# ChangUk/RecommenderSystems

Hardware: AMD Instinct MI355X
Metric: RWR seeds/sec + achieved HBM GB/s on 100M-edge bipartite graph, 1/2/4/8 GPUs (higher is better)
Workload: dtype f64

## Files before the change

### recommendersystems_amd/csrc/iterate.hip

```cpp
#include "iterate.h"

#include <climits>
#include <cstdlib>
#include <type_traits>

namespace rwr {

template <int G, bool VF>
__global__ __launch_bounds__(256) void k_spmm(int32_t n, const int64_t *__restrict__ in_ptr,
                                              const int32_t *__restrict__ in_src,
                                              const double *__restrict__ in_w,
                                              const int32_t *__restrict__ row_order, int32_t nrows,
                                              const double *__restrict__ X, double *__restrict__ Y,
                                              const int32_t *__restrict__ seeds, double c1, int skip_seed_row,
                                              const double *__restrict__ w_src, double *__restrict__ Zout)
{
    constexpr int RPW = WAVE / G;
    constexpr int U = 4;
    const int tile = blockIdx.y;
    const size_t toff = (size_t)tile * (size_t)n * G;
    X += toff;
    Y += toff;
    if (VF && Zout) Zout += toff;
    const int lane = threadIdx.x & (WAVE - 1);
    const int sub = lane / G, k = lane % G;
    const int32_t my_seed = skip_seed_row ? seeds[tile * G + k] : -1;
    const int wpb = blockDim.x / WAVE;
    const int64_t nwaves = (int64_t)gridDim.x * wpb;
    for (int64_t rb = ((int64_t)blockIdx.x * wpb + threadIdx.x / WAVE) * RPW; rb < nrows; rb += nwaves * RPW) {
        const int64_t r = rb + sub;
        int32_t j = -1;
        int64_t p = 0, e = 0;
        if (r < nrows) {
            j = row_order[r];
            p = in_ptr[j];
            e = in_ptr[j + 1];
        }
        double acc = 0.0;
        for (; p + U <= e; p += U) {
            int32_t idx[U];
            double wv[U], xv[U];
#pragma unroll
            for (int u = 0; u < U; ++u) idx[u] = in_src[p + u];
#pragma unroll
            for (int u = 0; u < U; ++u) wv[u] = VF ? 0.0 : in_w[p + u];
#pragma unroll
            for (int u = 0; u < U; ++u) xv[u] = X[(size_t)idx[u] * G + k];
#pragma unroll
            for (int u = 0; u < U; ++u) {
                if (VF) {
                    acc += xv[u];
                } else {
                    double rw = c1 * xv[u];
                    acc += rw * wv[u];
                }
            }
        }
        for (; p < e; ++p) {
            if (VF) {
                acc += X[(size_t)in_src[p] * G + k];
            } else {
                double rw = c1 * X[(size_t)in_src[p] * G + k];
                acc += rw * in_w[p];
            }
        }
        if (j >= 0 && j != my_seed) {
            Y[(size_t)j * G + k] = acc;
            if (VF && Zout) { const double rw = c1 * acc; Zout[(size_t)j * G + k] = rw * w_src[j]; }
        }
    }
}

template <int G, int CH, bool CHECK, bool WRITE, bool VF, bool SEL = false>
__device__ __forceinline__ void spmm_chunked_body(int32_t n, const int64_t *__restrict__ in_ptr,
                                                  const int32_t *__restrict__ in_src,
                                                  const double *__restrict__ in_w,
                                                  const int32_t *__restrict__ row_order, int32_t nrows,
                                                  const double *__restrict__ X, double *__restrict__ Y,
                                                  const int32_t *__restrict__ seeds, double c1,
                                                  int skip_seed_row, const uint32_t *__restrict__ nz_in,
                                                  uint32_t *__restrict__ nz_out,
                                                  const uint32_t *__restrict__ act,
                                                  const double *__restrict__ w_src, double *__restrict__ Zout,
                                                  const SelSink sink = SelSink{})
{
    static_assert(G >= 8 && G <= 64, "chunked SpMM needs 8 <= G <= 64");
    static_assert(!SEL || (!CHECK && !WRITE), "the selecting form probes and writes no bitmap");
    constexpr int RPW = WAVE / G;
    const int tile = blockIdx.y;
    const size_t toff = (size_t)tile * (size_t)n * G;
    X += toff;
    if (!SEL) Y += toff;
    if (VF && Zout) Zout += toff;
    const size_t nzw = ((size_t)n + 31) / 32;
    if (CHECK) nz_in += (size_t)tile * nzw;
    if (WRITE) nz_out += (size_t)tile * nzw;
    if (CHECK && act) act += (size_t)tile * nzw;
    const int lane = threadIdx.x & (WAVE - 1);
    const int sub = lane / G, k = lane % G;
    const int gbase = (lane - k) << 2;
    const int32_t my_seed = skip_seed_row ? seeds[tile * G + k] : -1;
    bool sel_real = false;
    double sel_tau = 0.0;
    if (SEL) {
        sel_real = seeds[tile * G + k] >= 0;
        sel_tau = sink.tau[tile * G + k];
    }
    const int wpb = blockDim.x / WAVE;
    const int64_t nwaves = (int64_t)gridDim.x * wpb;
    for (int64_t rb = ((int64_t)blockIdx.x * wpb + threadIdx.x / WAVE) * RPW; rb < nrows; rb += nwaves * RPW) {
        const int64_t r = rb + sub;
        int32_t j = -1;
        int64_t p = 0, e = 0;
        if (r < nrows) {
            j = row_order[r];
            p = in_ptr[j];
            e = in_ptr[j + 1];
            if (CHECK && act && !((act[(uint32_t)j >> 5] >> (j & 31)) & 1u)) e = p;
        }
        double acc = 0.0;
        while (__any(p < e)) {
            const int64_t left = e - p;
            const int cnt = left > CH ? CH : (left > 0 ? (int)left : 0);
            int32_t my_idx = 0;
            double my_w = 0.0;
            if (k < cnt) {
                my_idx = in_src[p + k];
                if (!VF) my_w = in_w[p + k];
                if (CHECK) {
                    const uint32_t wd = nz_in[(uint32_t)my_idx >> 5];
                    if (!((wd >> (my_idx & 31)) & 1u)) my_idx |= (int32_t)0x80000000;
                }
            }
            const int wlo = __double2loint(my_w), whi = __double2hiint(my_w);
            if (CHECK) {
                const unsigned long long lm = __ballot(k < cnt && my_idx >= 0);
                unsigned long long um = lm;
                if (G < 64) {
#pragma unroll
                    for (int sh = G; sh < 64; sh <<= 1) um |= um >> sh;
                    um &= (1ull << (G & 63)) - 1ull;
                }
                if (__popcll(um) <= 4) {
                    while (um) {
                        const int t = __builtin_ctzll(um);
                        um &= um - 1;
                        const int idx = __builtin_amdgcn_ds_bpermute(gbase + (t << 2), my_idx);
                        if (VF) {
                            if (t < cnt && idx >= 0) acc += X[(size_t)idx * G + k];
                        } else {
                            const int lo = __builtin_amdgcn_ds_bpermute(gbase + (t << 2), wlo);
                            const int hi = __builtin_amdgcn_ds_bpermute(gbase + (t << 2), whi);
                            if (t < cnt && idx >= 0) {
                                const double rw = c1 * X[(size_t)idx * G + k];
                                acc += rw * __hiloint2double(hi, lo);
                            }
                        }
                    }
                    p += cnt;
                    continue;
                }
            }
            double xv[CH], wv[CH];
#pragma unroll
            for (int t = 0; t < CH; ++t) {
                const int idx = __builtin_amdgcn_ds_bpermute(gbase + (t << 2), my_idx);
                if (!VF) {
                    const int lo = __builtin_amdgcn_ds_bpermute(gbase + (t << 2), wlo);
                    const int hi = __builtin_amdgcn_ds_bpermute(gbase + (t << 2), whi);
                    wv[t] = __hiloint2double(hi, lo);
                }
                xv[t] = (t < cnt && idx >= 0) ? X[(size_t)idx * G + k] : 0.0;
            }
#pragma unroll
            for (int t = 0; t < CH; ++t) {
                if (t < cnt) {
                    if (VF) {
                        acc += xv[t];
                    } else {
                        double rw = c1 * xv[t];
                        acc += rw * wv[t];
                    }
                }
            }
            p += cnt;
        }
        if constexpr (SEL) {
            if (j >= 0 && j != my_seed && sel_real && acc >= sel_tau) {
                const int slot = tile * G + k;
                const int32_t at = atomicAdd(&sink.cursor[slot], 1);
                if (at < sink.cap) sink.cand[(size_t)slot * (size_t)sink.stride + (size_t)at] = RowScore{j, 0, acc};
                else *sink.overflow = 1;
            }
        } else if (j >= 0 && j != my_seed) {
            Y[(size_t)j * G + k] = acc;
            if (VF && Zout) { const double rw = c1 * acc; Zout[(size_t)j * G + k] = rw * w_src[j]; }
        }
        if (WRITE) {
            const unsigned long long nzb = __ballot(acc != 0.0);
            const unsigned long long gmask = (G == 64) ? ~0ull : (((1ull << (G & 63)) - 1ull) << (sub * G));
            if (k == 0 && j >= 0 && (nzb & gmask)) atomicOr(&nz_out[(uint32_t)j >> 5], 1u << (j & 31));
        }
    }
}

template <int G, int CH, bool CHECK, bool WRITE, bool VF, bool LIST>
__global__ __launch_bounds__(256) void k_spmm_chunked(int32_t n, const int64_t *__restrict__ in_ptr,
                                                      const int32_t *__restrict__ in_src,
                                                      const double *__restrict__ in_w,
                                                      const int32_t *__restrict__ row_order, int32_t nrows,
                                                      const double *__restrict__ X, double *__restrict__ Y,
                                                      const int32_t *__restrict__ seeds, double c1,
                                                      int skip_seed_row, const uint32_t *__restrict__ nz_in,
                                                      uint32_t *__restrict__ nz_out,
                                                      const uint32_t *__restrict__ act,
                                                      const double *__restrict__ w_src, double *__restrict__ Zout)
{
    spmm_chunked_body<G, CH, CHECK, WRITE, VF>(n, in_ptr, in_src, in_w, row_order, nrows, X, Y, seeds, c1, skip_seed_row,
                                               nz_in, nz_out, act, w_src, Zout);
}

template <int G, int CH, bool VF>
__global__ __launch_bounds__(256) void k_spmm_select(int32_t n, const int64_t *__restrict__ in_ptr,
                                                     const int32_t *__restrict__ in_src,
                                                     const double *__restrict__ in_w,
                                                     const int32_t *__restrict__ rows, int32_t nrows,
                                                     const double *__restrict__ X, const int32_t *__restrict__ seeds,
                                                     double c1, const SelSink sink)
{
    if (sink.list) {
        rows = sink.list + (size_t)blockIdx.y * (size_t)sink.list_stride;
        nrows = sink.list_cnt[blockIdx.y];
    }
    spmm_chunked_body<G, CH, false, false, VF, true>(n, in_ptr, in_src, in_w, rows, nrows, X, nullptr, seeds, c1, 1, nullptr,
                                                     nullptr, nullptr, nullptr, nullptr, sink);
}

template <int G, int CH, bool VF>
__global__ __launch_bounds__(256) void k_spmm_frontier(int32_t n, const int64_t *__restrict__ in_ptr,
                                                       const int32_t *__restrict__ in_src,
                                                       const double *__restrict__ in_w,
                                                       const int32_t *__restrict__ fl_rows,
                                                       const int32_t *__restrict__ fl_cnt,
                                                       const double *__restrict__ X, double *__restrict__ Y,
                                                       const int32_t *__restrict__ seeds, double c1,
                                                       int skip_seed_row, const uint32_t *__restrict__ nz_in,
                                                       uint32_t *__restrict__ nz_out,
                                                       const double *__restrict__ w_src, double *__restrict__ Zout)
{
    const int tile = blockIdx.y;
    spmm_chunked_body<G, CH, true, true, VF>(n, in_ptr, in_src, in_w, fl_rows + (size_t)tile * (size_t)n, fl_cnt[tile], X, Y,
                                             seeds, c1, skip_seed_row, nz_in, nz_out, nullptr, w_src, Zout);
}

__global__ __launch_bounds__(256) void k_mark_active(int32_t n, const uint32_t *__restrict__ nz, uint32_t *__restrict__ act,
                                                     const int64_t *__restrict__ rowptr, const int32_t *__restrict__ dst,
                                                     const uint8_t *__restrict__ etype, int G, const int32_t *__restrict__ seeds,
                                                     int32_t *__restrict__ fl_rows, int32_t *__restrict__ fl_cnt)
{
    const size_t nzw = ((size_t)n + 31) / 32;
    const int tile = blockIdx.y;
    const int lane = threadIdx.x & (WAVE - 1);
    const size_t wi = (size_t)blockIdx.x * (blockDim.x / WAVE) + threadIdx.x / WAVE;
    uint32_t *a = act + (size_t)tile * nzw;
    int32_t *list = fl_rows ? fl_rows + (size_t)tile * (size_t)n : nullptr;
    if (list && blockIdx.x == 0 && threadIdx.x < (unsigned)G) {
        const int32_t sr = seeds[tile * G + threadIdx.x];
        if (sr >= 0) {
            const uint32_t bit = 1u << (sr & 31);
            if (!(atomicOr(&a[(uint32_t)sr >> 5], bit) & bit)) list[atomicAdd(&fl_cnt[tile], 1)] = sr;
        }
    }
    if (wi >= nzw) return;
    uint32_t w = nz[(size_t)tile * nzw + wi];
    while (w) {
        const int b = __builtin_ctz(w);
        w &= w - 1;
        const int64_t i = (int64_t)wi * 32 + b;
        const int64_t p1 = rowptr[i + 1];
        if (!list) {
            for (int64_t p = rowptr[i] + lane; p < p1; p += WAVE)
                if (etype[p] != RWR_EDGE_UNDEFINED) {
                    const int32_t t = dst[p];
                    atomicOr(&a[(uint32_t)t >> 5], 1u << (t & 31));
                }
            continue;
        }
        for (int64_t p0 = rowptr[i]; p0 < p1; p0 += WAVE) {
            const int64_t p = p0 + lane;
            bool add = false;
            int32_t t = 0;
            if (p < p1 && etype[p] != RWR_EDGE_UNDEFINED) {
                t = dst[p];
                const uint32_t bit = 1u << (t & 31);
                add = !(atomicOr(&a[(uint32_t)t >> 5], bit) & bit);
            }
            const unsigned long long m = __ballot(add);
            if (!m) continue;
            const int leader = __builtin_ctzll(m);
            int base = 0;
            if (lane == leader) base = atomicAdd(&fl_cnt[tile], (int)__popcll(m));
            base = __shfl(base, leader);
            const int below = __builtin_amdgcn_mbcnt_hi((uint32_t)(m >> 32), __builtin_amdgcn_mbcnt_lo((uint32_t)m, 0u));
            if (add) list[base + below] = t;
        }
    }
}

template <int G>
__global__ __launch_bounds__(64) void k_seed_chain(int32_t n, int ntiles, const int64_t *__restrict__ in_ptr,
                                                   const int32_t *__restrict__ in_src,
                                                   const double *__restrict__ in_w,
                                                   const uint8_t *__restrict__ dangling,
                                                   const double *__restrict__ X, double *__restrict__ Y,
                                                   const int32_t *__restrict__ seeds, double c1,
                                                   uint32_t *__restrict__ nz_out)
{
    constexpr int U = 8;
    const int q = blockIdx.x * blockDim.x + threadIdx.x;
    if (q >= ntiles * G) return;
    const int tile = q / G, k = q % G;
    const int32_t s = seeds[q];
    if (s < 0) return;
    const double *x = X + (size_t)tile * (size_t)n * G + k;
    int64_t p = in_ptr[s];
    const int64_t e = in_ptr[s + 1];
    int32_t nxt = (p < e) ? in_src[p] : INT_MAX;
    double acc = 0.0;
    int32_t i = 0;
    for (; i + U <= n; i += U) {
        double xv[U];
        uint8_t dg[U];
#pragma unroll
        for (int u = 0; u < U; ++u) xv[u] = x[(size_t)(i + u) * G];
#pragma unroll
        for (int u = 0; u < U; ++u) dg[u] = dangling[i + u];
#pragma unroll
        for (int u = 0; u < U; ++u) {
            double rw = c1 * xv[u];
            while (nxt == i + u) {
                acc += rw * in_w[p];
                ++p;
                nxt = (p < e) ? in_src[p] : INT_MAX;
            }
            acc += dg[u] ? xv[u] : (xv[u] - rw);
        }
    }
    for (; i < n; ++i) {
        double xi = x[(size_t)i * G];
        double rw = c1 * xi;
        while (nxt == i) {
            acc += rw * in_w[p];
            ++p;
            nxt = (p < e) ? in_src[p] : INT_MAX;
        }
        acc += dangling[i] ? xi : (xi - rw);
    }
    Y[(size_t)tile * (size_t)n * G + (size_t)s * G + k] = acc;
    if (nz_out && acc != 0.0)
        atomicOr(&nz_out[(size_t)tile * (((size_t)n + 31) / 32) + ((uint32_t)s >> 5)], 1u << (s & 31));
}

__global__ void k_gate(const unsigned int *__restrict__ gate, unsigned int expected)
{
    const long long t0 = __builtin_amdgcn_s_memrealtime();
    while (__hip_atomic_load(gate, __ATOMIC_RELAXED, __HIP_MEMORY_SCOPE_AGENT) < expected) {
        if (__builtin_amdgcn_s_memrealtime() - t0 > 100000) break;
        __builtin_amdgcn_s_sleep(32);
    }
}

template <int G, bool VF>
__global__ __launch_bounds__(256) void k_seed_terms(int32_t n, const int64_t *__restrict__ in_ptr,
                                                    const int32_t *__restrict__ in_src,
                                                    const double *__restrict__ in_w, const double *__restrict__ X,
                                                    const int32_t *__restrict__ seeds, double c1,
                                                    const int64_t *__restrict__ evoff, double *__restrict__ evterm,
                                                    const uint32_t *__restrict__ nz)
{
    const int slot = blockIdx.y;
    const int32_t s = seeds[slot];
    if (s < 0) return;
    const int tile = slot / G, k = slot % G;
    const double *x = X + (size_t)tile * (size_t)n * G + k;
    const int64_t p0 = in_ptr[s], deg = in_ptr[s + 1] - p0;
    double *out = evterm + evoff[slot];
    if (nz) nz += (size_t)tile * (((size_t)n + 31) / 32);
    for (int64_t q = (int64_t)blockIdx.x * blockDim.x + threadIdx.x; q < deg; q += (int64_t)gridDim.x * blockDim.x) {
        const int32_t i = in_src[p0 + q];
        if (nz && !((nz[(uint32_t)i >> 5] >> (i & 31)) & 1u)) {
            out[q] = 0.0;
        } else if (VF) {
            out[q] = x[(size_t)i * G];
        } else {
            const double rw = c1 * x[(size_t)i * G];
            out[q] = rw * in_w[p0 + q];
        }
    }
}

template <int G>
__global__ __launch_bounds__(64) void k_seed_chain_sparse(int32_t n, const int64_t *__restrict__ in_ptr,
                                                          const int32_t *__restrict__ in_src,
                                                          const uint8_t *__restrict__ dangling,
                                                          const double *__restrict__ X, double *__restrict__ Y,
                                                          const int32_t *__restrict__ seeds, double c1,
                                                          const int64_t *__restrict__ evoff,
                                                          const double *__restrict__ evterm,
                                                          const uint32_t *__restrict__ nz_x, uint32_t *__restrict__ nz_out,
                                                          unsigned int *__restrict__ gate)
{
    if (threadIdx.x == 0 && gate) __hip_atomic_fetch_add(gate, 1u, __ATOMIC_RELAXED, __HIP_MEMORY_SCOPE_AGENT);
    const int tile = blockIdx.x, lane = threadIdx.x;
    const size_t nzw = ((size_t)n + 31) / 32;
    const uint32_t *bits = nz_x + (size_t)tile * nzw;
    const double *x = X + (size_t)tile * (size_t)n * G;
    const bool consumer = lane < G;
    const int k = lane % G;
    int32_t s = -1;
    int64_t p = 0, e = 0;
    const double *termp = evterm;
    if (consumer) {
        s = seeds[tile * G + k];
        if (s >= 0) {
            p = in_ptr[s];
            e = in_ptr[s + 1];
            termp = evterm + evoff[tile * G + k] - p;
        }
    }
    double acc = 0.0;
    for (size_t w0 = 0; w0 < nzw; w0 += WAVE) {
        const uint32_t word = (w0 + lane < nzw) ? bits[w0 + lane] : 0u;
        unsigned long long mask = __ballot(word != 0u);
        while (mask) {
            const int l = __builtin_ctzll(mask);
            mask &= mask - 1;
            uint32_t wv = (uint32_t)__builtin_amdgcn_readlane((int)word, l);
            while (wv) {
                const int b = __builtin_ctz(wv);
                wv &= wv - 1;
                const int32_t i = (int32_t)((w0 + l) * 32 + b);
                if (consumer && s >= 0) {
                    while (p < e && in_src[p] < i) ++p;
                    while (p < e && in_src[p] == i) { acc += termp[p]; ++p; }
                    const double xi = x[(size_t)i * G + k];
                    const double rw = c1 * xi;
                    acc += dangling[i] ? xi : (xi - rw);
                }
            }
        }
    }
    if (consumer && s >= 0) {
        Y[(size_t)tile * (size_t)n * G + (size_t)s * G + k] = acc;
        if (nz_out && acc != 0.0)
            atomicOr(&nz_out[(size_t)tile * nzw + ((uint32_t)s >> 5)], 1u << (s & 31));
    }
}

constexpr int CH3_NSW = 6;
constexpr int CH3_NST = CH3_NSW * WAVE;
constexpr int CH3_LPT = 16;
constexpr int CH3_CE = CH3_NST * CH3_LPT;
template <int G, bool MASK>
__global__ __launch_bounds__(WAVE + CH3_NST) void k_seed_chain_roles(
    int32_t n, const int64_t *__restrict__ in_ptr, const int32_t *__restrict__ in_src,
    const uint8_t *__restrict__ dangling, const double *__restrict__ X, double *__restrict__ Y,
    const int32_t *__restrict__ seeds, double c1, const int64_t *__restrict__ evoff,
    const double *__restrict__ evterm, uint32_t *__restrict__ nz_out, unsigned int *__restrict__ gate,
    const uint32_t *__restrict__ nz_x)
{
    if (threadIdx.x == 0 && gate) __hip_atomic_fetch_add(gate, 1u, __ATOMIC_RELAXED, __HIP_MEMORY_SCOPE_AGENT);
    constexpr int CR = CH3_CE / G;
    static_assert(CR % 32 == 0, "chunk rows must be a multiple of 32");
    extern __shared__ double rr[];
    const int tile = blockIdx.x;
    const double *x = X + (size_t)tile * (size_t)n * G;
    const int tid = threadIdx.x;
    const int64_t total = (int64_t)n * G;
    const int nchunks = (int)((total + CH3_CE - 1) / CH3_CE);
    if (MASK) nz_x += (size_t)tile * (((size_t)n + 31) / 32);

    if (tid >= WAVE) {
        const int st = tid - WAVE;
        double rega[CH3_LPT], regb[CH3_LPT];
        uint8_t dga[CH3_LPT], dgb[CH3_LPT];
        constexpr int NW = MASK ? CR / 32 : 1;
        uint32_t bwa[NW], bwb[NW];
        const int64_t nzw = ((int64_t)n + 31) / 32;
#define CH3_LOAD(R, D, W, C)                                                    \
    {                                                                           \
        const int64_t base__ = (int64_t)(C) * CH3_CE;                           \
        _Pragma("unroll") for (int u = 0; u < CH3_LPT; ++u) {                   \
            int64_t el = base__ + (int64_t)u * CH3_NST + st;                    \
            el = el < total ? el : total - 1;                                   \
            R[u] = x[el];                                                       \
            D[u] = dangling[el / G];                                            \
        }                                                                       \
        if (MASK) {                                                             \
            _Pragma("unroll") for (int j = 0; j < NW; ++j) {                    \
                int64_t wi__ = (int64_t)(C) * (CR / 32) + j;                    \
                wi__ = wi__ < nzw ? wi__ : nzw - 1;  \
                W[j] = nz_x[wi__];                                              \
            }                                                                   \
        }                                                                       \
    }
#define CH3_STAGE(R, D, W, C)                                                                           \
    {                                                                                                   \
        const int64_t base__ = (int64_t)(C) * CH3_CE;                                                   \
        double *buf__ = rr + (size_t)((C) & 1) * CH3_CE;                                                \
        _Pragma("unroll") for (int u = 0; u < CH3_LPT; ++u) {                                           \
            const int off = u * CH3_NST + st;                                                           \
            bool live__ = base__ + off < total;                                                         \
            if (MASK) {  \
                const int row__ = off / G, j0__ = (u * CH3_NST / G) >> 5;                               \
                uint32_t wd__ = W[j0__];                                                                \
                _Pragma("unroll") for (int dj = 1; dj <= 2; ++dj)                                       \
                    if (j0__ + dj < NW && (row__ >> 5) == j0__ + dj) wd__ = W[j0__ + dj < NW ? j0__ + dj : 0]; \
                live__ = live__ && ((wd__ >> (row__ & 31)) & 1u);                                       \
            }                                                                                           \
            const double xv = live__ ? R[u] : 0.0;  \
            const double rw = c1 * xv;                                                                  \
            buf__[off] = D[u] ? xv : (xv - rw);                                                         \
        }                                                                                               \
    }
        static_assert(!MASK || (CH3_NST - 1) / G + 1 <= 64, "a thread's value of one load lies at most two bitmap words on");
        CH3_LOAD(rega, dga, bwa, 0)
        if (nchunks > 1) CH3_LOAD(regb, dgb, bwb, 1)
        for (int c = 0; c < nchunks; c += 2) {
            CH3_STAGE(rega, dga, bwa, c)
            if (c + 2 < nchunks) CH3_LOAD(rega, dga, bwa, c + 2)
            __builtin_amdgcn_fence(__ATOMIC_RELEASE, "workgroup", "local");
            __builtin_amdgcn_s_barrier();
            if (c + 1 < nchunks) {
                CH3_STAGE(regb, dgb, bwb, c + 1)
                if (c + 3 < nchunks) CH3_LOAD(regb, dgb, bwb, c + 3)
                __builtin_amdgcn_fence(__ATOMIC_RELEASE, "workgroup", "local");
                __builtin_amdgcn_s_barrier();
            }
        }
#undef CH3_LOAD
#undef CH3_STAGE
        return;
    }

    const bool consumer = tid < G;
    const int k = tid % G;
    int32_t s = -1;
    int64_t p = 0, e = 0;
    const int32_t *srcp = in_src;
    const double *termp = evterm;
    int32_t nxt = INT_MAX, raw_s = INT_MAX;
    double tcur = 0.0, raw_t = 0.0;
    bool has2 = false;
    if (consumer) {
        s = seeds[tile * G + k];
        if (s >= 0) {
            p = in_ptr[s];
            e = in_ptr[s + 1];
            termp = evterm + evoff[tile * G + k] - p;
            if (p < e) { nxt = srcp[p]; tcur = termp[p]; ++p; }
            if (p < e) { raw_s = srcp[p]; raw_t = termp[p]; has2 = true; ++p; }
        }
    }
    double acc = 0.0;
    __builtin_amdgcn_s_setprio(3);
    for (int c = 0; c < nchunks; ++c) {
        __builtin_amdgcn_s_barrier();
        __builtin_amdgcn_fence(__ATOMIC_ACQUIRE, "workgroup", "local");
        const double *buf = rr + (size_t)(c & 1) * CH3_CE;
        const int64_t row0 = (int64_t)c * CR;
#define CH3_READ(V, R0) _Pragma("unroll") for (int u = 0; u < 32; ++u) V[u] = buf[((R0) + u) * G + k];
#define CH3_FOLD(V, R0)                                                                                     \
    {                                                                                                       \
        const bool evt = __any(consumer && nxt < row0 + (R0) + 32);                                         \
        if (!evt) {                                                                                         \
            _Pragma("unroll") for (int u = 0; u < 32; ++u) acc += V[u];                                     \
        } else {                                                                                            \
            _Pragma("unroll") for (int u = 0; u < 32; ++u) {                                                \
                const int32_t i = (int32_t)(row0 + (R0)) + u;                                               \
                if (__any(consumer && nxt == i)) {                                                          \
                    while (consumer && nxt == i) {                                                          \
                        acc += tcur;                                                                        \
                        nxt = has2 ? raw_s : INT_MAX;  \
                        tcur = raw_t;                                                                       \
                        has2 = p < e;                 \
                        const int64_t pc = has2 ? p : e - 1;                                                \
                        raw_s = srcp[pc];                                                                   \
                        raw_t = termp[pc];                                                                  \
                        p += has2 ? 1 : 0;                                                                  \
                    }                                                                                       \
                }                                                                                           \
                acc += V[u];                            \
            }                                                                                               \
        }                                                                                                   \
    }
        double ra[32], rb[32];
        CH3_READ(ra, 0)
#pragma unroll 1
        for (int r0 = 0; r0 + 64 <= CR; r0 += 64) {
            CH3_READ(rb, r0 + 32)
            CH3_FOLD(ra, r0)
            if (r0 + 64 < CR) CH3_READ(ra, r0 + 64)
            CH3_FOLD(rb, r0 + 32)
        }
        if (CR % 64 != 0) CH3_FOLD(ra, CR - 32)
#undef CH3_READ
#undef CH3_FOLD
    }
    __builtin_amdgcn_s_setprio(0);
    if (consumer && s >= 0) {
        Y[(size_t)tile * (size_t)n * G + (size_t)s * G + k] = acc;
        if (nz_out && acc != 0.0)
            atomicOr(&nz_out[(size_t)tile * (((size_t)n + 31) / 32) + ((uint32_t)s >> 5)], 1u << (s & 31));
    }
}

__global__ void k_init_seeds(int32_t n, int ntiles, int G, double *__restrict__ X,
                             const int32_t *__restrict__ seeds, uint32_t *__restrict__ nz,
                             double *__restrict__ Z = nullptr, const double *__restrict__ w_src = nullptr, double c1 = 0.0)
{
    const int q = blockIdx.x * blockDim.x + threadIdx.x;
    if (q >= ntiles * G) return;
    const int32_t s = seeds[q];
    if (s < 0) return;
    const int tile = q / G;
    const size_t row = (size_t)tile * (size_t)n * G + (size_t)s * G;
    const double rw = c1 * (double)n;
    const double zs = Z ? rw * w_src[s] : 0.0;
    for (int kk = 0; kk < G; ++kk) {
        const bool mine = seeds[tile * G + kk] == s;
        X[row + kk] = mine ? (double)n : 0.0;
        if (Z) Z[row + kk] = mine ? zs : 0.0;
    }
    if (nz) atomicOr(&nz[(size_t)tile * (((size_t)n + 31) / 32) + ((uint32_t)s >> 5)], 1u << (s & 31));
}

__global__ void k_seed_z(int32_t n, int ntiles, int G, const double *__restrict__ Y, double *__restrict__ Z,
                         const int32_t *__restrict__ seeds, const double *__restrict__ w_src, double c1)
{
    const int q = blockIdx.x * blockDim.x + threadIdx.x;
    if (q >= ntiles * G) return;
    const int32_t s = seeds[q];
    if (s < 0) return;
    const size_t at = (size_t)(q / G) * (size_t)n * G + (size_t)s * G + (q % G);
    const double rw = c1 * Y[at];
    Z[at] = rw * w_src[s];
}
__global__ __launch_bounds__(256) void k_make_z(int64_t elems, int G, const double *__restrict__ X, double *__restrict__ Z,
                                                const double *__restrict__ w_src, double c1)
{
    const int64_t q = (int64_t)blockIdx.x * blockDim.x + threadIdx.x;
    if (q >= elems) return;
    const double rw = c1 * X[q];
    Z[q] = rw * w_src[q / G];
}

__global__ __launch_bounds__(256) void k_make_z_nz(int32_t lo, int32_t hi, int G, const double *__restrict__ X, double *__restrict__ Zs,
                                                   const double *__restrict__ w_src, double c1, uint32_t *__restrict__ nz)
{
    const int64_t j = ((int64_t)lo & ~(int64_t)63) + (int64_t)blockIdx.x * blockDim.x + threadIdx.x;
    bool any = false;
    if (j >= lo && j < hi) {
        const double w = w_src[j];
        const size_t at = (size_t)(j - lo) * G;
        for (int k = 0; k < G; ++k) {
            const double xv = X[(size_t)j * G + k];
            const double rw = c1 * xv;
            Zs[at + k] = rw * w;
            any = any || xv != 0.0;
        }
    }
    const unsigned long long m = __ballot(any);
    const int lane = threadIdx.x & (WAVE - 1);
    if (lane == 0 && (uint32_t)m) nz[(uint64_t)j >> 5] = (uint32_t)m;
    if (lane == 32 && (uint32_t)(m >> 32)) nz[(uint64_t)j >> 5] = (uint32_t)(m >> 32);
}


static PlanInput read_plan_knobs()
{
    PlanInput v;
    const char *e;
    if ((e = getenv("RWR_SPMM"))) v.spmm = atoi(e);
    if ((e = RWR_TUNE_ENV("RWR_NZ_ITERS"))) v.nz_iters = atoi(e);
    if ((e = getenv("RWR_ACT_ITERS"))) v.act_iters = atoi(e);
    if ((e = RWR_TUNE_ENV("RWR_ACT_MIN_N"))) v.act_min_n = atol(e);
    if ((e = getenv("RWR_FRONTIER_LIST"))) v.frontier_list = atoi(e);
    if ((e = getenv("RWR_CHAIN"))) v.chain = atoi(e);
    if ((e = RWR_TUNE_ENV("RWR_SCAN_WORK"))) v.scan_work = atof(e);
    if ((e = RWR_TUNE_ENV("RWR_SCAN_SIDE"))) v.scan_side = atoi(e);
    if ((e = RWR_TUNE_ENV("RWR_GATE"))) v.gate = atoi(e);
    if ((e = getenv("RWR_TAIL_ROWS"))) v.tail_rows = atoi(e);
    if ((e = RWR_TUNE_ENV("RWR_CHAIN_SERIAL"))) v.two_streams = atoi(e) == 0;
    if ((e = getenv("RWR_X_CLEAR"))) v.x_clear = atoi(e);
    return v;
}
static const PlanInput &plan_knobs() { static const PlanInput k = read_plan_knobs(); return k; }

template <class F> static void bool_dispatch(F &&f) { f(); }
template <class F, class... B> static void bool_dispatch(F &&f, bool b, B... bs)
{
    bool_dispatch([&](auto... c) { if (b) f(std::true_type{}, c...); else f(std::false_type{}, c...); }, bs...);
}

template <int G>
static void launch_spmm_g(rwr_graph *g, int tg, const SpmmArgs &a, hipStream_t s)
{
    const bool vf = a.Zin != nullptr;
    const double *GS = vf ? a.Zin : a.X;
    const int skip = a.skip_seed_row;
    constexpr int RPW = WAVE / G;
    constexpr int CH = G > 16 ? 16 : G;
    if constexpr (G >= 8) {
        if (a.rows.kind == Rows::Frontier) {
            const int32_t *fl_rows = g->fl_rows.p, *fl_cnt = g->fl_rows.p + (size_t)tg * (size_t)g->n;
            const unsigned want = cdiv((size_t)g->n / 10 + 1, (size_t)RPW * 4);
            const unsigned gx = want < 1u ? 1u : want < 2048u ? want : 2048u;
            bool_dispatch([&](auto v) {
                hipLaunchKernelGGL((k_spmm_frontier<G, CH, decltype(v)::value>), dim3(gx, tg), dim3(256), 0, s, g->n, g->in_ptr.p,
                                   g->in_src.p, g->in_w.p, fl_rows, fl_cnt, GS, a.Y, a.seeds, a.c1, skip, a.nz_in, a.nz_out,
                                   g->w_src.p, a.Zout);
            }, vf);
            return;
        }
    }
    const bool listed = a.rows.kind == Rows::Tail;
    const int32_t *order = listed ? g->tail_rows[a.rows.level].p : g->row_order.p;
    int32_t nrows = listed ? g->tail_n[a.rows.level] : g->n;
    if (listed) {
        const int32_t first = a.row_first < nrows ? a.row_first : nrows;
        order += first;
        nrows = (a.row_count >= 0 && a.row_count < nrows - first) ? a.row_count : nrows - first;
    }
    if (nrows <= 0 && (a.sel || a.row_count >= 0)) return;
    unsigned want = cdiv((size_t)nrows, (size_t)RPW * 4);
    unsigned gx = want < 1u ? 1u : want < 8192u ? want : 8192u;
    if constexpr (G == 1) {
        if (tg == 1 && plan_knobs().spmm != 0) {
            launch_spmv_exact(g, a.X, a.Y, a.seeds, a.c1, skip, a.act, a.nz_out, s, a.Zin, a.Zout, a.hub_scan);
            return;
        }
    }
    if constexpr (G >= 8) {
        if (a.sel) {
            const SelSink sink = *a.sel;
            bool_dispatch([&](auto v) {
                hipLaunchKernelGGL((k_spmm_select<G, CH, decltype(v)::value>), dim3(gx, tg), dim3(256), 0, s, g->n, g->in_ptr.p,
                                   g->in_src.p, g->in_w.p, order, nrows, GS, a.seeds, a.c1, sink);
            }, vf);
            return;
        }
    }
    if constexpr (G >= 8) {
        if (plan_knobs().spmm != 0) {
            bool_dispatch([&](auto chk, auto wr, auto v, auto lst) {
                if constexpr (decltype(chk)::value || !decltype(wr)::value)
                    hipLaunchKernelGGL((k_spmm_chunked<G, CH, decltype(chk)::value, decltype(wr)::value, decltype(v)::value,
                                                       decltype(lst)::value>), dim3(gx, tg), dim3(256), 0, s, g->n, g->in_ptr.p,
                                       g->in_src.p, g->in_w.p, order, nrows, GS, a.Y, a.seeds, a.c1, skip, a.nz_in, a.nz_out,
                                       a.act, g->w_src.p, a.Zout);
            }, a.nz_in != nullptr, a.nz_in && a.nz_out, vf, listed);
            return;
        }
    }
    bool_dispatch([&](auto v) {
        hipLaunchKernelGGL((k_spmm<G, decltype(v)::value>), dim3(gx, tg), dim3(256), 0, s, g->n, g->in_ptr.p, g->in_src.p,
                           g->in_w.p, order, nrows, GS, a.Y, a.seeds, a.c1, skip, g->w_src.p, a.Zout);
    }, vf);
}
void launch_spmm(rwr_graph *g, int G, int tg, const SpmmArgs &a, hipStream_t s)
{
    RWR_DISPATCH_G(G, launch_spmm_g<GG>(g, tg, a, s));
}
void launch_init_seeds(rwr_graph *g, int G, int tg, double *X, const int32_t *seeds, uint32_t *nz, double *Z, double c1,
                       hipStream_t s)
{
    hipLaunchKernelGGL(k_init_seeds, dim3(cdiv((size_t)tg * G, 64)), dim3(64), 0, s, g->n, tg, G, X, seeds, nz, Z, g->w_src.p, c1);
}
void launch_make_z(int64_t elems, int G, const double *X, double *Z, const double *w_src, double c1, hipStream_t s)
{
    hipLaunchKernelGGL(k_make_z, dim3(cdiv((size_t)elems, 256)), dim3(256), 0, s, elems, G, X, Z, w_src, c1);
}
void launch_make_z_nz(rwr_graph *g, int32_t lo, int32_t hi, int G, const double *X, double *Zs, double c1, uint32_t *nz,
                      hipStream_t s)
{
    const int64_t first = (int64_t)lo & ~(int64_t)63;
    hipLaunchKernelGGL(k_make_z_nz, dim3(cdiv((size_t)((int64_t)hi - first), 256)), dim3(256), 0, s, lo, hi, G, X, Zs, g->w_src.p,
                       c1, nz);
}
void launch_mark_active(rwr_graph *g, int G, int tg, const uint32_t *nz, uint32_t *act, const int32_t *seeds, int32_t *fl_rows,
                        int32_t *fl_cnt, hipStream_t s)
{
    const size_t nzw = ((size_t)g->n + 31) / 32;
    hipLaunchKernelGGL(k_mark_active, dim3(cdiv(nzw, 4), tg), dim3(256), 0, s, g->n, nz, act, g->rowptr.p, g->dst.p, g->etype.p,
                       G, seeds, fl_rows, fl_cnt);
}
template <int G>
static void launch_seed_terms(rwr_graph *g, int tg, const double *X, const int32_t *seeds, double c1,
                              const int64_t *evoff, hipStream_t s, const double *Zin, const uint32_t *nz = nullptr)
{
    const unsigned term_blocks = g->max_in_deg > 256 * 8 ? 8u : cdiv((size_t)(g->max_in_deg > 0 ? g->max_in_deg : 1), 256);
    bool_dispatch([&](auto v) {
        hipLaunchKernelGGL((k_seed_terms<G, decltype(v)::value>), dim3(term_blocks, tg * G), dim3(256), 0, s, g->n, g->in_ptr.p,
                           g->in_src.p, g->in_w.p, Zin ? Zin : X, seeds, c1, evoff, g->d_evterm.p, nz);
    }, Zin != nullptr);
}
template <int G>
static void launch_chain(rwr_graph *g, int tg, const double *X, double *Y, const int32_t *seeds, double c1,
                         const int64_t *evoff, uint32_t *nz_out, unsigned int *gate, hipStream_t s,
                         Chain kind, const uint32_t *nz_x, bool masked)
{
    if (kind == Chain::Sparse) {
        hipLaunchKernelGGL(k_seed_chain_sparse<G>, dim3(tg), dim3(64), 0, s, g->n, g->in_ptr.p, g->in_src.p,
                           g->dangling.p, X, Y, seeds, c1, evoff, g->d_evterm.p, nz_x, nz_out, gate);
        return;
    }
    if (kind == Chain::Roles) {
        constexpr size_t smem = 2 * CH3_CE * sizeof(double);
        bool_dispatch([&](auto m) {
            constexpr bool MASK = decltype(m)::value && G >= 8;
            (void)hipFuncSetAttribute((const void *)k_seed_chain_roles<G, MASK>, hipFuncAttributeMaxDynamicSharedMemorySize,
                                      (int)smem);
            hipLaunchKernelGGL((k_seed_chain_roles<G, MASK>), dim3(tg), dim3(WAVE + CH3_NST), smem, s, g->n, g->in_ptr.p,
                               g->in_src.p, g->dangling.p, X, Y, seeds, c1, evoff, g->d_evterm.p, nz_out, gate, nz_x);
        }, masked);
        return;
    }
    hipLaunchKernelGGL(k_seed_chain<G>, dim3(cdiv((size_t)tg * G, 64)), dim3(64), 0, s, g->n, tg, g->in_ptr.p,
                       g->in_src.p, g->in_w.p, g->dangling.p, X, Y, seeds, c1, nz_out);
}

int32_t Profile::record(hipEvent_t &e, hipStream_t s)
{
    e = nullptr;
    if (!on) return RWR_OK;
    if (used == pool.size()) { RWR_HIP(hipEventCreate(&e)); pool.push_back(e); }
    e = pool[used++];
    RWR_HIP(hipEventRecord(e, s));
    return RWR_OK;
}
int32_t Profile::end(std::vector<hipEvent_t> &stage, hipEvent_t a, hipStream_t s)
{
    hipEvent_t b; RWR_TRY(record(b, s));
    if (on) stage.insert(stage.end(), {a, b});
    return RWR_OK;
}
int32_t Profile::fold(rwr_graph *g)
{
    auto drain = [&](const std::vector<hipEvent_t> &v, double *acc, bool dense_only) -> int32_t {
        for (size_t i = 0; i + 1 < v.size(); i += 2) {
            float ms = 0.f;
            if (dense_only && !dense[i / 2]) continue;
            RWR_HIP(hipEventElapsedTime(&ms, v[i], v[i + 1]));
            *acc += ms;
        }
        return RWR_OK;
    };
    if (on) {
        RWR_TRY(drain(spmm, &g->stats.spmm_dense_ms, true));
        RWR_TRY(drain(spmm, &g->stats.spmm_ms, false));
        RWR_TRY(drain(chain, &g->stats.chain_ms, false));
        RWR_TRY(drain(rank, &g->stats.rank_ms, false));
        RWR_TRY(drain(iter, &g->stats.iterate_wall_ms, false));
        RWR_TRY(drain(bound, &g->stats.rank_bound_ms, false));
    }
    reset();
    return RWR_OK;
}

int32_t GroupIter::init(bool fresh, bool ranks_nonneg, bool ranking_only)
{
    const int32_t n = g->n;
    hipStream_t s = g->stream;
    const size_t elems = (size_t)tg * (size_t)n * G;
    PlanInput in = plan_knobs();
    in.n = n; in.nnz = g->nnz; in.nonneg = g->nonneg; in.big_n = spmv_big_n(); in.seed_row_kernel = g->opts.seed_row_kernel;
    in.scan_self = chain_scan_self_contained(G); in.G = G; in.tg = tg; in.c1 = c1;
    in.fresh = fresh; in.ranks_nonneg = ranks_nonneg; in.ranking_only = ranking_only;
    cfg = plan_config(in);
    if (!fresh && Zc) launch_make_z((int64_t)elems, G, X, Zc, g->w_src.p, c1, s);
    const size_t nzw = ((size_t)n + 31) / 32;
    if (cfg.flist && g->fl_rows.ensure((size_t)tg * (size_t)n + (size_t)tg) != RWR_OK) {
        (void)hipGetLastError();
        cfg.flist = false;
        cfg.clear_x = plan_clear_x(cfg);
    }
    if (fresh && cfg.clear_x) RWR_HIP(hipMemsetAsync(X, 0, elems * sizeof(double), s));
    if (fresh && !cfg.clear_x) g->stats.x_clear_skipped += 1;
    if (fresh && Zc && !cfg.flist) RWR_HIP(hipMemsetAsync(Zc, 0, elems * sizeof(double), s));
    nz_cur = cfg.nz_iters > 0 ? g->d_nz.p : nullptr;
    nz_oth = cfg.nz_iters > 0 ? g->d_nz.p + (size_t)tg * nzw : nullptr;
    if (nz_cur) RWR_HIP(hipMemsetAsync(nz_cur, 0, (size_t)tg * nzw * sizeof(uint32_t), s));
    if (fresh) launch_init_seeds(g, G, tg, X, d_seeds, nz_cur, Zc, c1, s);
    RWR_HIP(hipGetLastError());
    if (cfg.scan) RWR_TRY(chain_scan_prepare(g, G, tg, d_seeds, s));
    if (Zc && G == 1 && tg == 1 && cfg.addends_nonneg) RWR_TRY(sweep_prepare(g));
    if (Zc && cfg.chain_kind == 0 && !cfg.scan) RWR_TRY(ensure_in_w(g));
    return RWR_OK;
}

int32_t GroupIter::step(const StepPlan &p, Profile &prof, int32_t row_first, int32_t row_count)
{
    const int32_t n = g->n;
    hipStream_t s = g->stream;
    const size_t nzw = ((size_t)n + 31) / 32;
    constexpr int GATE_SLOTS = 64;
    const uint32_t *nz_in = p.probe ? nz_cur : nullptr;
    uint32_t *nz_out = p.write_bits ? nz_oth : nullptr;
    if (nz_out) RWR_HIP(hipMemsetAsync(nz_out, 0, (size_t)tg * nzw * sizeof(uint32_t), s));
    uint32_t *act = p.mark ? g->d_nz.p + 2 * (size_t)tg * nzw : nullptr;
    const bool listed = p.rows.kind == Rows::Frontier;
    if (act) {
        int32_t *fl_rows = listed ? g->fl_rows.p : nullptr, *fl_cnt = listed ? fl_rows + (size_t)tg * (size_t)n : nullptr;
        RWR_HIP(hipMemsetAsync(act, 0, (size_t)tg * nzw * sizeof(uint32_t), s));
        if (fl_cnt) RWR_HIP(hipMemsetAsync(fl_cnt, 0, (size_t)tg * sizeof(int32_t), s));
        launch_mark_active(g, G, tg, nz_in, act, d_seeds, fl_rows, fl_cnt, s);
    }
    const uint32_t *nz_terms = p.terms_nz ? nz_in : nullptr;
    double *zout = (Zc && p.form_z) ? Zn : nullptr;
    hipStream_t sc = p.chain_side ? g->stream2 : s;
    unsigned int *gate_it = p.gate ? g->d_gate.p + (it % GATE_SLOTS) : nullptr;
    if (p.chain != Chain::None) {
        if (!p.scan()) RWR_DISPATCH_G(G, launch_seed_terms<GG>(g, tg, X, d_seeds, c1, d_evoff, s, Zc, nz_terms));
        if (gate_it) RWR_HIP(hipMemsetAsync(gate_it, 0, sizeof(unsigned int), s));
        if (p.chain_side) { RWR_HIP(hipEventRecord(g->ev_fork, s)); RWR_HIP(hipStreamWaitEvent(sc, g->ev_fork, 0)); }
        if (p.scan() && !(p.chain_self && Zc)) RWR_DISPATCH_G(G, launch_seed_terms<GG>(g, tg, X, d_seeds, c1, d_evoff, sc, Zc, nz_terms));
        hipEvent_t c0; RWR_TRY(prof.record(c0, sc));
        if (p.scan())
            RWR_TRY(chain_scan_step(g, G, tg, X, Y, d_seeds, d_evoff, c1, nz_out, sc, p.chain_self ? Zc : nullptr,
                                    p.chain_self ? zout : nullptr));
        else
            RWR_DISPATCH_G(G, launch_chain<GG>(g, tg, X, Y, d_seeds, c1, d_evoff, nz_out, gate_it, sc, p.chain, nz_in,
                                                       p.chain_masked));
        RWR_TRY(prof.end(prof.chain, c0, sc));
        if (p.chain_side) RWR_HIP(hipEventRecord(g->ev_join, sc));
    }
    if (gate_it) hipLaunchKernelGGL(k_gate, dim3(1), dim3(1), 0, s, gate_it, (unsigned)(tg < 192 ? tg : 192));
    hipEvent_t a; RWR_TRY(prof.record(a, s));
    SpmmArgs sp;
    sp.X = X, sp.Y = Y, sp.seeds = d_seeds, sp.c1 = c1, sp.skip_seed_row = true;
    sp.nz_in = nz_in, sp.nz_out = nz_out, sp.act = act, sp.Zin = Zc, sp.Zout = zout;
    sp.hub_scan = cfg.addends_nonneg, sp.rows = p.rows;
    sp.row_first = row_first, sp.row_count = row_count;
    launch_spmm(g, G, tg, sp, s);
    RWR_TRY(prof.end(prof.spmm, a, s));
    if (prof.on) prof.dense.push_back(p.dense());
    if (p.dense()) { g->stats.spmm_dense_launches += 1; ++dense_steps; }
    if (p.chain_side) RWR_HIP(hipStreamWaitEvent(s, g->ev_join, 0));
    if (zout && p.seed_z) hipLaunchKernelGGL(k_seed_z, dim3(cdiv((size_t)tg * G, 64)), dim3(64), 0, s, n, tg, G, Y, zout, d_seeds, g->w_src.p, c1);
    RWR_HIP(hipGetLastError());
    { double *t = X; X = Y; Y = t; }
    { double *t = Zc; Zc = Zn; Zn = t; }
    { uint32_t *tz = nz_cur; nz_cur = nz_oth; nz_oth = tz; }
    g->stats.spmm_launches += 1;
    g->stats.chain_launches += p.chain != Chain::None; g->stats.frontier_list_launches += listed;
    ++it;
    return RWR_OK;
}

int32_t GroupIter::redo_rows(const StepPlan &p, Profile &prof, int32_t row_first, int32_t row_count, const SelSink *sel)
{
    hipStream_t s = g->stream;
    hipEvent_t a; RWR_TRY(prof.record(a, s));
    SpmmArgs sp;
    sp.X = Y, sp.Y = X, sp.seeds = d_seeds, sp.c1 = c1, sp.skip_seed_row = true;
    sp.Zin = Zn, sp.Zout = nullptr;
    sp.hub_scan = cfg.addends_nonneg, sp.rows = p.rows;
    sp.row_first = row_first, sp.row_count = row_count, sp.sel = sel;
    launch_spmm(g, G, tg, sp, s);
    RWR_TRY(prof.end(prof.spmm, a, s));
    if (prof.on) prof.dense.push_back(0);
    RWR_HIP(hipGetLastError());
    return RWR_OK;
}

int32_t iterate_group(rwr_graph *g, int G, int tg, const int32_t *d_seeds, const int64_t *d_evoff, const int32_t *h_seeds,
                      double d, int64_t T, Profile &prof, double **final_X, int64_t *dense_steps, SplitLast *split)
{
    GroupIter gi(g, G, tg, d_seeds, d_evoff, d);
    RWR_TRY(gi.init(true, true, T >= 1));
    if (gi.cfg.tails) {
        RWR_TRY(tail_rows_prepare(g));
        gi.cfg.tail_depth = g->tail_depth;
        for (size_t q = 0; q < (size_t)tg * G; ++q)
            if (h_seeds[q] >= 0) gi.cfg.need |= g->h_tail_flag[h_seeds[q]];
    }
    bool split_ok = false;
    if (split && split->head > 0 && T >= 1 && G >= 8 && plan_knobs().spmm != 0) {
        const StepPlan last = plan_step(gi.cfg, T - 1, T);
        split_ok = last.rows.kind == Rows::Tail && last.rows.level == 0 && !last.probe && !last.write_bits && !last.form_z &&
                   last.chain == Chain::None;
        split->last = last;
    }
    while (gi.it < T) {
        const StepPlan p = plan_step(gi.cfg, gi.it, T);
        if (split_ok && gi.it == T - 1) RWR_TRY(gi.step(p, prof, 0, split->head));
        else RWR_TRY(gi.step(p, prof));
    }
    if (split_ok) { split->taken = true; split->gi.emplace(gi); }
    *final_X = gi.X;
    *dense_steps = gi.dense_steps;
    return RWR_OK;
}

}
```

Baseline: 847.0.

## Load wider aligned index/weight batches and consume them in CH-sized gather rounds

The chunked SpMM loop now loads up to LW edge indices and weights per iteration (G lanes, or 32 in the VF case at G=64) instead of CH. It then runs several CH-wide gather rounds from that single load, with an early exit when no lane has work left. Load starts are aligned to LW boundaries via the new spmm_next_load helper, which is meant to give coalesced, aligned index/weight reads and fewer loop trips. In exchange it adds per-round __any checks, and for G=64 unrolling may raise register pressure.

```diff
diff --git a/recommendersystems_amd/csrc/iterate.hip b/recommendersystems_amd/csrc/iterate.hip
--- a/recommendersystems_amd/csrc/iterate.hip
+++ b/recommendersystems_amd/csrc/iterate.hip
@@ -1,4 +1,5 @@
 #include "iterate.h"
+#include "spmm_chunk.h"
 
 #include <climits>
 #include <cstdlib>
@@ -87,6 +88,8 @@
     static_assert(G >= 8 && G <= 64, "chunked SpMM needs 8 <= G <= 64");
     static_assert(!SEL || (!CHECK && !WRITE), "the selecting form probes and writes no bitmap");
     constexpr int RPW = WAVE / G;
+    constexpr int LW = G <= 32 ? G : VF ? 32 : CH;
+    static_assert(LW % CH == 0 && CH <= LW, "an index load is a whole number of gather rounds");
     const int tile = blockIdx.y;
     const size_t toff = (size_t)tile * (size_t)n * G;
     X += toff;
@@ -120,8 +123,7 @@
         }
         double acc = 0.0;
         while (__any(p < e)) {
-            const int64_t left = e - p;
-            const int cnt = left > CH ? CH : (left > 0 ? (int)left : 0);
+            const int cnt = spmm_next_load(p, e - p, LW);
             int32_t my_idx = 0;
             double my_w = 0.0;
             if (k < cnt) {
@@ -133,53 +135,59 @@
                 }
             }
             const int wlo = __double2loint(my_w), whi = __double2hiint(my_w);
+            unsigned long long um = 0;
             if (CHECK) {
-                const unsigned long long lm = __ballot(k < cnt && my_idx >= 0);
-                unsigned long long um = lm;
+                um = __ballot(k < cnt && my_idx >= 0);
                 if (G < 64) {
 #pragma unroll
                     for (int sh = G; sh < 64; sh <<= 1) um |= um >> sh;
                     um &= (1ull << (G & 63)) - 1ull;
                 }
-                if (__popcll(um) <= 4) {
-                    while (um) {
-                        const int t = __builtin_ctzll(um);
-                        um &= um - 1;
-                        const int idx = __builtin_amdgcn_ds_bpermute(gbase + (t << 2), my_idx);
-                        if (VF) {
-                            if (t < cnt && idx >= 0) acc += X[(size_t)idx * G + k];
-                        } else {
-                            const int lo = __builtin_amdgcn_ds_bpermute(gbase + (t << 2), wlo);
-                            const int hi = __builtin_amdgcn_ds_bpermute(gbase + (t << 2), whi);
-                            if (t < cnt && idx >= 0) {
-                                const double rw = c1 * X[(size_t)idx * G + k];
-                                acc += rw * __hiloint2double(hi, lo);
+            }
+#pragma unroll G == 64 ? LW / CH : 1
+            for (int r0 = 0; r0 < LW; r0 += CH) {
+                if (r0 > 0 && !__any(cnt > r0)) break;
+                if (CHECK) {
+                    unsigned long long rm = (um >> r0) & ((1ull << CH) - 1ull);
+                    if (__popcll(rm) <= 4) {
+                        while (rm) {
+                            const int t = r0 + __builtin_ctzll(rm);
+                            rm &= rm - 1;
+                            const int idx = __builtin_amdgcn_ds_bpermute(gbase + (t << 2), my_idx);
+                            if (VF) {
+                                if (t < cnt && idx >= 0) acc += X[(size_t)idx * G + k];
+                            } else {
+                                const int lo = __builtin_amdgcn_ds_bpermute(gbase + (t << 2), wlo);
+                                const int hi = __builtin_amdgcn_ds_bpermute(gbase + (t << 2), whi);
+                                if (t < cnt && idx >= 0) {
+                                    const double rw = c1 * X[(size_t)idx * G + k];
+                                    acc += rw * __hiloint2double(hi, lo);
+                                }
                             }
                         }
+                        continue;
                     }
-                    p += cnt;
-                    continue;
                 }
-            }
-            double xv[CH], wv[CH];
+                double xv[CH], wv[CH];
 #pragma unroll
-            for (int t = 0; t < CH; ++t) {
-                const int idx = __builtin_amdgcn_ds_bpermute(gbase + (t << 2), my_idx);
-                if (!VF) {
-                    const int lo = __builtin_amdgcn_ds_bpermute(gbase + (t << 2), wlo);
-                    const int hi = __builtin_amdgcn_ds_bpermute(gbase + (t << 2), whi);
-                    wv[t] = __hiloint2double(hi, lo);
+                for (int t = 0; t < CH; ++t) {
+                    const int idx = __builtin_amdgcn_ds_bpermute(gbase + ((r0 + t) << 2), my_idx);
+                    if (!VF) {
+                        const int lo = __builtin_amdgcn_ds_bpermute(gbase + ((r0 + t) << 2), wlo);
+                        const int hi = __builtin_amdgcn_ds_bpermute(gbase + ((r0 + t) << 2), whi);
+                        wv[t] = __hiloint2double(hi, lo);
+                    }
+                    xv[t] = (r0 + t < cnt && idx >= 0) ? X[(size_t)idx * G + k] : 0.0;
                 }
-                xv[t] = (t < cnt && idx >= 0) ? X[(size_t)idx * G + k] : 0.0;
-            }
 #pragma unroll
-            for (int t = 0; t < CH; ++t) {
-                if (t < cnt) {
-                    if (VF) {
-                        acc += xv[t];
-                    } else {
-                        double rw = c1 * xv[t];
-                        acc += rw * wv[t];
+                for (int t = 0; t < CH; ++t) {
+                    if (r0 + t < cnt) {
+                        if (VF) {
+                            acc += xv[t];
+                        } else {
+                            double rw = c1 * xv[t];
+                            acc += rw * wv[t];
+                        }
                     }
                 }
             }
diff --git a/recommendersystems_amd/csrc/spmm_chunk.h b/recommendersystems_amd/csrc/spmm_chunk.h
--- /dev/null
+++ b/recommendersystems_amd/csrc/spmm_chunk.h
@@ -0,0 +1,18 @@
+#pragma once
+
+#include <cstdint>
+
+#if defined(__HIPCC__) || defined(__CUDACC__)
+#define RWR_CHUNK_HD __host__ __device__
+#else
+#define RWR_CHUNK_HD
+#endif
+
+namespace rwr {
+
+constexpr RWR_CHUNK_HD int spmm_next_load(int64_t p, int64_t left, int LW)
+{
+    return left <= 0 ? 0 : left <= LW ? (int)left : LW - (int)(p & (int64_t)(LW - 1));
+}
+
+}
```

Result: faster. 866.2 (median of 6 runs) (+2.3%).
